# jyf588/SimGAN

Hardware: AMD Instinct MI355X
Metric: env-steps/sec of GAIL-dyn PPO update (higher is better)
Workload: dtype f32; 1 GPU; northstar: GAIL-dyn update, T=128 N=512/GPU obs=47 act=12 D-in=86 policy=mlp h64 D h100 ppo_epoch=10 num_mini_batch=1...; optimizer_steps_per_update=2720, parallelism=single GPU

## Files before the change

### simgan_amd/csrc/sg_disc_step4.hpp

```cpp
#pragma once

struct Step4Args {
    PregatherArgs next;
    double* loss_acc;
};

#define SG_STEP4_TIMEOUT_TICKS 300000000ll

__device__ __forceinline__ float sg_ld_sc1(__amdgpu_buffer_rsrc_t r, int byte_off) {
    return __uint_as_float(__builtin_amdgcn_raw_buffer_load_b32(r, byte_off, 0, 16 ));
}

__device__ __forceinline__ bool sg_step4_wait(const unsigned* flags, int lo, int hi, unsigned want, int lane) {
    const long long deadline = wall_clock64() + SG_STEP4_TIMEOUT_TICKS;
    for (int it = 0;; ++it) {
        bool ok = true;
        for (int j = lo + lane; j < hi; j += 64) ok = ok & (__hip_atomic_load(flags + j * SG_STEP4_FLAG_STRIDE, __ATOMIC_RELAXED, __HIP_MEMORY_SCOPE_AGENT) == want);
        if (__all(ok)) return true;
        if ((it & 31) == 31 && wall_clock64() > deadline) return false;
        __builtin_amdgcn_s_sleep(1);
    }
}

template <int KF, int KH>
__global__ __launch_bounds__(512) void k_disc_step4(float* c_params, float* c_m, float* c_v, float* c_wT, float* c_ops,
                                                   SgOptState* c_st, int c_pack ,
                                                   int c_B, Step4Args a) {
    constexpr int Fp = 16 * KF, Hp = 16 * KH, ldF = Fp + 4, ldH = Hp + 4;
    constexpr int NWC = KF > KH ? KF : KH;
    constexpr int W_LDS = 8 * 256, C_LDS = SG_CHAIN4_LDS_FLOATS(KF, KH);
    __shared__ __attribute__((aligned(16))) float sm[(C_LDS > W_LDS ? C_LDS : W_LDS) + 4];
    const int c_G = c_pack & 1023, c_k1 = (int)((unsigned)c_pack >> 14);
    const int tid = threadIdx.x, wave = tid >> 6, lane = tid & 63;
    const int Kt = 64 * c_G, n_chain = 12 * c_G, w_base = (n_chain + 7) & ~7;
    unsigned* flags = reinterpret_cast<unsigned*>(c_st) + SG_STEP4_FLAG_WORD0;
    float* c_part = c_ops + (size_t)(2 - ((c_k1 - 1) & 1)) * ((size_t)Kt * (3 * Hp + ldF + Fp));

    if ((int)blockIdx.x < n_chain) {
        if (wave >= NWC) return;
        int t0 = 0;
        if (tid == 0) t0 = c_st->t0;
        Chain4Args ca{c_params, c_wT, c_ops, c_part, c_B, c_G, 1.0f / (float)c_B, 10.0f};
        sg_chain4_body<KF, KH, true>(ca, sm);
        asm volatile("s_waitcnt vmcnt(0)" ::: "memory");
        __syncthreads();
        if (tid == 0) __hip_atomic_store(flags + blockIdx.x * SG_STEP4_FLAG_STRIDE, (unsigned)(t0 + c_k1), __ATOMIC_RELAXED, __HIP_MEMORY_SCOPE_AGENT);
        return;
    }
    const int wb = (int)blockIdx.x - w_base;
    constexpr int th = KH, tf = KF, T2 = th * th, ntv = 8 * (th + tf), NV = (3 * Hp + 4 + 63) / 64;
    static_assert((8 - th) * (th + tf) > NV, "k_disc_step4: a spare slot must exist for the Adam-scalar lane");
    if (wb < 0) return;
    if (wb >= ntv) {
        if (a.next.ops) sg_disc_pregather(a.next, wb - ntv);
        return;
    }
    SgDiscDesc d;
    d.F = 0; d.Hd = 0; d.Hp = Hp; d.Fp = Fp; d.ldF = ldF; d.ldH = ldH;
    d.w1 = 0; d.b1 = Hp * ldF; d.w2 = d.b1 + Hp; d.b2 = d.w2 + Hp * ldH; d.w3 = d.b2 + Hp; d.b3 = d.w3 + Hp; d.total = d.b3 + 16;
    float (*red)[256] = reinterpret_cast<float (*)[256]>(sm);
    int* sh_ok = reinterpret_cast<int*>(sm + W_LDS);
    unsigned* err = reinterpret_cast<unsigned*>(c_st) + SG_STEP4_ERR_WORD;
    const int xcd = wb & 7, slot = wb >> 3;
    const int li = lane & 15, lq = lane >> 4;
    constexpr int nw = 8;
    if (xcd < th) {
        const int b = slot < th ? xcd * th + slot : T2 + xcd * tf + (slot - th);
        const bool w2 = b < T2;
        const int t = w2 ? b : b - T2;
        const int tm = w2 ? t / th : t / tf, tn = w2 ? t % th : t % tf;
        const int ldp = w2 ? ldH : ldF;
        const int idx = (w2 ? d.w2 : d.w1) + (tm * 16 + ((tid & 255) >> 4)) * ldp + tn * 16 + (tid & 15);
        float p0 = 0.f, m0 = 0.f, v0 = 0.f;
        float4 sc = float4{0.f, 0.f, 1.f, 1.f};
        int t0 = 0;
        if (tid < 256) {
            p0 = c_params[idx]; m0 = c_m[idx]; v0 = c_v[idx];
            sc = *reinterpret_cast<const float4*>(c_st->step_size2);
        }
        if (tid < 256 || wave == 7) t0 = c_st->t0;
        const SgStacks stk = sg_disc_stacks(c_ops, Kt, Hp, Fp, ldF);
        const float* L = (w2 ? stk.L2 : stk.L1) + (size_t)tm * Kt * 16;
        const float* Rr = (w2 ? stk.R2 : stk.R1t) + (size_t)tn * Kt * 16;
        const int n_chunks = Kt >> 4;
        const __amdgpu_buffer_rsrc_t rL = __builtin_amdgcn_make_buffer_rsrc(const_cast<float*>(L), 0, Kt * 64, 0x00020000);
        const __amdgpu_buffer_rsrc_t rR = __builtin_amdgcn_make_buffer_rsrc(const_cast<float*>(Rr), 0, Kt * 64, 0x00020000);
        int img0 = 0, img1 = 0;
        sg_disc_img_pos(d, w2, tm * 16 + ((tid & 255) >> 4), tn * 16 + (tid & 15), img0, img1);
        if (tid == 0) *sh_ok = 1;
        __syncthreads();
        const unsigned want = (unsigned)(t0 + c_k1);
        if (wave == 7 && (__hip_atomic_load(err, __ATOMIC_RELAXED, __HIP_MEMORY_SCOPE_AGENT) != 0 || !sg_step4_wait(flags, 4 * c_G, n_chain, want, lane)) && lane == 0) *sh_ok = 0;
        __syncthreads();
        if (!*sh_ok) { if (tid == 0) { atomicOr(err, 1u); a.loss_acc[0] = __builtin_nanf(""); } return; }
        f32x4 acc = f32x4{0.f, 0.f, 0.f, 0.f}, alt = acc;
        const int half_chunks = n_chunks >> 1;
        auto contract = [&](int c_lo, int c_hi, auto&& between) {
            bool first = true;
            for (int c0 = c_lo + wave; c0 < c_hi || first; c0 += 2 * nw) {
                float x[2][4], y[2][4];
#pragma unroll
                for (int cc = 0; cc < 2; ++cc)
#pragma unroll
                    for (int s = 0; s < 4; ++s) {
                        const int c = c0 + cc * nw;
                        const int r = c < c_hi ? 16 * c + 4 * s + lq : Kt;
                        x[cc][s] = sg_ld_sc1(rL, (r * 16 + li) * 4);
                        y[cc][s] = sg_ld_sc1(rR, (r * 16 + li) * 4);
                    }
                if (first) { between(); first = false; }
#pragma unroll
                for (int cc = 0; cc < 2; ++cc)
#pragma unroll
                    for (int s = 0; s < 4; ++s) {
                        if (s & 1) alt = sg_mfma(x[cc][s], y[cc][s], alt);
                        else acc = sg_mfma(x[cc][s], y[cc][s], acc);
                    }
            }
        };
        contract(0, half_chunks, [&]() {
            if (wave == 7 && !sg_step4_wait(flags, 0, 4 * c_G, want, lane) && lane == 0) *sh_ok = 0;
        });
        __syncthreads();
        if (!*sh_ok) { if (tid == 0) { atomicOr(err, 1u); a.loss_acc[0] = __builtin_nanf(""); } return; }
        contract(half_chunks, n_chunks, []() {});
        acc += alt;
#pragma unroll
        for (int r = 0; r < 4; ++r) red[wave][(4 * lq + r) * 16 + li] = acc[r];
        __syncthreads();
        if (tid < 256) {
            float g = 0.f;
            {
                float r8[8];
#pragma unroll
                for (int w = 0; w < 8; ++w) r8[w] = red[w][tid];
#pragma unroll
                for (int w = 0; w < 8; ++w) g += r8[w];
            }
            const bool odd = (t0 + c_k1) & 1;
            const float step_size = odd ? sc.y : sc.x, bc2_sqrt = odd ? sc.w : sc.z;
            m0 = m0 + (g - m0) * (float)(1.0 - 0.9);
            v0 = v0 * (float)0.999 + (float)(1.0 - 0.999) * g * g;
            const float denom = sqrtf(v0) / bc2_sqrt + SG_DISC_ADAM_EPS;
            p0 = p0 - step_size * (m0 / denom);
            __builtin_amdgcn_sched_barrier(0);
            __builtin_nontemporal_store(p0, c_params + idx);
            __builtin_nontemporal_store(m0, c_m + idx);
            __builtin_nontemporal_store(v0, c_v + idx);
            __builtin_nontemporal_store(p0, c_wT + img0);
            __builtin_nontemporal_store(p0, c_wT + img1);
        }
        return;
    }
    const int vid = (xcd - th) * (th + tf) + slot;
    if (vid > NV) return;
    if (vid == NV) {
        if (tid == 0) sg_opt_prepare(c_st, c_st->t0 + c_k1 + 1);
        return;
    }
    {
        const int nparts = n_chain, stride = 4 * Hp, NE = 3 * Hp + 4;
        const int i = 64 * vid + lane;
        const float4 sc = *reinterpret_cast<const float4*>(c_st->step_size2);
        const int t0 = c_st->t0;
        const bool odd = (t0 + c_k1) & 1;
        const float step_size = odd ? sc.y : sc.x, bc2_sqrt = odd ? sc.w : sc.z;
        const bool is_param = wave == 0 && i < 3 * Hp + 1;
        const int pidx = i < Hp ? d.b1 + i : i < 2 * Hp ? d.b2 + (i - Hp) : i < 3 * Hp ? d.w3 + (i - 2 * Hp) : d.b3;
        float pv = 0.f, pm = 0.f, pvv = 0.f;
        if (is_param) { pv = c_params[pidx]; pm = c_m[pidx]; pvv = c_v[pidx]; }
        const __amdgpu_buffer_rsrc_t rP = __builtin_amdgcn_make_buffer_rsrc(c_part, 0, nparts * stride * 4, 0x00020000);
        if (tid == 0) *sh_ok = 1;
        __syncthreads();
        if (wave == 7 && (__hip_atomic_load(err, __ATOMIC_RELAXED, __HIP_MEMORY_SCOPE_AGENT) != 0 || !sg_step4_wait(flags, 0, n_chain, (unsigned)(t0 + c_k1), lane)) && lane == 0) *sh_ok = 0;
        __syncthreads();
        if (!*sh_ok) { if (tid == 0) { atomicOr(err, 1u); a.loss_acc[0] = __builtin_nanf(""); } return; }
        float g = 0.f;
        if (i < NE) {
            for (int s0 = wave; s0 < nparts; s0 += 16 * nw) {
                float tt[16];
#pragma unroll
                for (int u = 0; u < 16; ++u) {
                    const int sidx = s0 + u * nw;
                    tt[u] = sidx < nparts ? sg_ld_sc1(rP, (sidx * stride + i) * 4) : 0.f;
                }
#pragma unroll
                for (int u = 0; u < 16; ++u) g += tt[u];
            }
        }
        red[wave][lane] = g;
        __syncthreads();
        if (wave == 0 && i < NE) {
            g = 0.f;
            {
                float r8[8];
#pragma unroll
                for (int w = 0; w < 8; ++w) r8[w] = red[w][lane];
#pragma unroll
                for (int w = 0; w < 8; ++w) g += r8[w];
            }
            if (i < 3 * Hp + 1) {
                pm = pm + (g - pm) * (float)(1.0 - 0.9);
                pvv = pvv * (float)0.999 + (float)(1.0 - 0.999) * g * g;
                const float denom = sqrtf(pvv) / bc2_sqrt + SG_DISC_ADAM_EPS;
                c_params[pidx] = pv - step_size * (pm / denom);
                c_m[pidx] = pm;
                c_v[pidx] = pvv;
            }
            const int l0 = (3 * Hp) & 63;
            const float el_s = __shfl(g, l0 + 1), pl_s = __shfl(g, l0 + 2), gp_s = __shfl(g, l0 + 3);
            if (i == 3 * Hp) {
                const float inv_B = 1.0f / (float)c_B;
                const float el = el_s * inv_B, pl = pl_s * inv_B, gp = 10.0f * (gp_s * inv_B);
                a.loss_acc[0] += (double)(el + pl + gp);
                a.loss_acc[1] += (double)el;
                a.loss_acc[2] += (double)pl;
            }
        }
    }
}
```

Measured before the change: 2.489 million env-steps/s.

## Split flag polling across two waves and prefetch contraction batches before waits

Wave 6 now polls the second flag group (after a short delay, using pipelined sc1 global loads) while wave 7 polls the first, and the two report through workgroup-scope LDS words instead of block-wide __syncthreads. Other waves spin on those words, issue their first operand loads as soon as the first group is ready, and then load the second batch, so global latency overlaps the cross-block wait. The second half's chunk assignment is rotated per wave. This adds inline-asm polling, spin loops on LDS words and more register pressure from the held prefetch buffers.

```diff
diff --git a/simgan_amd/csrc/sg_disc_step4.hpp b/simgan_amd/csrc/sg_disc_step4.hpp
--- a/simgan_amd/csrc/sg_disc_step4.hpp
+++ b/simgan_amd/csrc/sg_disc_step4.hpp
@@ -20,6 +20,40 @@
         if ((it & 31) == 31 && wall_clock64() > deadline) return false;
         __builtin_amdgcn_s_sleep(1);
     }
+}
+
+#define SG_STEP4_POLLS 1
+#define SG_STEP4_POLL_START_TICKS 340
+struct SgStep4Polls { unsigned r[SG_STEP4_POLLS] = {}; };
+__device__ __forceinline__ unsigned sg_step4_poll(const unsigned* p) {
+    unsigned r;
+    asm volatile("global_load_dword %0, %1, off sc1" : "=v"(r) : "v"(p) : "memory");
+    return r;
+}
+__device__ __forceinline__ bool sg_step4_wait_piped(SgStep4Polls& pp, const unsigned* flags, int n, unsigned want, int lane, const int* quit) {
+    constexpr int K = SG_STEP4_POLLS;
+    static_assert(K >= 1 && K <= 3, "SG_STEP4_POLLS: 1, 2 or 3");
+    const unsigned* p = flags + (lane < n ? lane : n - 1) * SG_STEP4_FLAG_STRIDE;
+    const long long deadline = wall_clock64() + SG_STEP4_TIMEOUT_TICKS;
+#pragma unroll
+    for (int i = 0; i < K; ++i) {
+        pp.r[i] = sg_step4_poll(p);
+        if (i + 1 < K) __builtin_amdgcn_s_sleep(28 / K);
+    }
+    for (int it = 0;; ++it) {
+#pragma unroll
+        for (int i = 0; i < K; ++i) {
+            asm volatile("s_waitcnt vmcnt(%1)" : "+v"(pp.r[i]) : "n"(K - 1) : "memory");
+            if (__all(pp.r[i] == want)) return true;
+            __builtin_amdgcn_s_sleep(1);
+            pp.r[i] = sg_step4_poll(p);
+        }
+        if ((it & 31) == 31 && (wall_clock64() > deadline || __hip_atomic_load(quit, __ATOMIC_RELAXED, __HIP_MEMORY_SCOPE_WORKGROUP) == 2)) return false;
+    }
+}
+__device__ __forceinline__ void sg_step4_polls_retire(SgStep4Polls& pp) {
+#pragma unroll
+    for (int i = 0; i < SG_STEP4_POLLS; ++i) asm volatile("" : "+v"(pp.r[i]) : : "memory");
 }
 
 template <int KF, int KH>
@@ -78,7 +112,7 @@
             p0 = c_params[idx]; m0 = c_m[idx]; v0 = c_v[idx];
             sc = *reinterpret_cast<const float4*>(c_st->step_size2);
         }
-        if (tid < 256 || wave == 7) t0 = c_st->t0;
+        if (tid < 256 || wave >= 6) t0 = c_st->t0;
         const SgStacks stk = sg_disc_stacks(c_ops, Kt, Hp, Fp, ldF);
         const float* L = (w2 ? stk.L2 : stk.L1) + (size_t)tm * Kt * 16;
         const float* Rr = (w2 ? stk.R2 : stk.R1t) + (size_t)tn * Kt * 16;
@@ -87,46 +121,92 @@
         const __amdgpu_buffer_rsrc_t rR = __builtin_amdgcn_make_buffer_rsrc(const_cast<float*>(Rr), 0, Kt * 64, 0x00020000);
         int img0 = 0, img1 = 0;
         sg_disc_img_pos(d, w2, tm * 16 + ((tid & 255) >> 4), tn * 16 + (tid & 15), img0, img1);
-        if (tid == 0) *sh_ok = 1;
+        const int half_chunks = n_chunks >> 1;
+        auto batch_offs = [&](int c0, int c_hi, int (&o)[2][4]) {
+#pragma unroll
+            for (int cc = 0; cc < 2; ++cc)
+#pragma unroll
+                for (int s = 0; s < 4; ++s) {
+                    const int c = c0 + cc * nw;
+                    const int r = c < c_hi ? 16 * c + 4 * s + lq : Kt;
+                    o[cc][s] = (r * 16 + li) * 4;
+                }
+        };
+        const int mix0 = half_chunks + ((wave - half_chunks) & (nw - 1));
+        int oa[2][4], ob[2][4];
+        batch_offs(wave, half_chunks, oa);
+        batch_offs(mix0, n_chunks, ob);
+#pragma unroll
+        for (int cc = 0; cc < 2; ++cc)
+#pragma unroll
+            for (int s = 0; s < 4; ++s) asm volatile("" : "+v"(oa[cc][s]), "+v"(ob[cc][s]));
+        int* sh_bce = sh_ok + 1;
+        int* sh_mix = sh_ok + 2;
+        if (tid == 0) { *sh_bce = 0; *sh_mix = 0; }
+        const long long poll_from = wall_clock64() + SG_STEP4_POLL_START_TICKS;
         __syncthreads();
         const unsigned want = (unsigned)(t0 + c_k1);
-        if (wave == 7 && (__hip_atomic_load(err, __ATOMIC_RELAXED, __HIP_MEMORY_SCOPE_AGENT) != 0 || !sg_step4_wait(flags, 4 * c_G, n_chain, want, lane)) && lane == 0) *sh_ok = 0;
-        __syncthreads();
-        if (!*sh_ok) { if (tid == 0) { atomicOr(err, 1u); a.loss_acc[0] = __builtin_nanf(""); } return; }
+        auto word_set = [&](int* w, bool up) {
+            if (lane == 0) __hip_atomic_store(w, up ? 1 : 2, __ATOMIC_RELAXED, __HIP_MEMORY_SCOPE_WORKGROUP);
+        };
+        auto word_up = [&](int* w) -> bool {
+            int s;
+            while ((s = __hip_atomic_load(w, __ATOMIC_RELAXED, __HIP_MEMORY_SCOPE_WORKGROUP)) == 0) __builtin_amdgcn_s_sleep(1);
+            asm volatile("" ::: "memory");
+            return s == 1;
+        };
+        SgStep4Polls pp;
+        if (wave == 7) {
+            word_set(sh_bce, __hip_atomic_load(err, __ATOMIC_RELAXED, __HIP_MEMORY_SCOPE_AGENT) == 0 && sg_step4_wait(flags, 4 * c_G, n_chain, want, lane));
+        } else if (wave == 6) {
+            bool up = __hip_atomic_load(err, __ATOMIC_RELAXED, __HIP_MEMORY_SCOPE_AGENT) == 0;
+            if (up) {
+                while (wall_clock64() < poll_from) __builtin_amdgcn_s_sleep(2);
+                up = 4 * c_G <= 64 ? sg_step4_wait_piped(pp, flags, 4 * c_G, want, lane, sh_bce) : sg_step4_wait(flags, 0, 4 * c_G, want, lane);
+            }
+            word_set(sh_mix, up);
+        }
         f32x4 acc = f32x4{0.f, 0.f, 0.f, 0.f}, alt = acc;
-        const int half_chunks = n_chunks >> 1;
-        auto contract = [&](int c_lo, int c_hi, auto&& between) {
-            bool first = true;
-            for (int c0 = c_lo + wave; c0 < c_hi || first; c0 += 2 * nw) {
-                float x[2][4], y[2][4];
-#pragma unroll
-                for (int cc = 0; cc < 2; ++cc)
-#pragma unroll
-                    for (int s = 0; s < 4; ++s) {
-                        const int c = c0 + cc * nw;
-                        const int r = c < c_hi ? 16 * c + 4 * s + lq : Kt;
-                        x[cc][s] = sg_ld_sc1(rL, (r * 16 + li) * 4);
-                        y[cc][s] = sg_ld_sc1(rR, (r * 16 + li) * 4);
-                    }
-                if (first) { between(); first = false; }
-#pragma unroll
-                for (int cc = 0; cc < 2; ++cc)
-#pragma unroll
-                    for (int s = 0; s < 4; ++s) {
-                        if (s & 1) alt = sg_mfma(x[cc][s], y[cc][s], alt);
-                        else acc = sg_mfma(x[cc][s], y[cc][s], acc);
-                    }
-            }
-        };
-        contract(0, half_chunks, [&]() {
-            if (wave == 7 && !sg_step4_wait(flags, 0, 4 * c_G, want, lane) && lane == 0) *sh_ok = 0;
-        });
-        __syncthreads();
-        if (!*sh_ok) { if (tid == 0) { atomicOr(err, 1u); a.loss_acc[0] = __builtin_nanf(""); } return; }
-        contract(half_chunks, n_chunks, []() {});
+        auto load_offs = [&](const int (&o)[2][4], float (&x)[2][4], float (&y)[2][4]) {
+#pragma unroll
+            for (int cc = 0; cc < 2; ++cc)
+#pragma unroll
+                for (int s = 0; s < 4; ++s) {
+                    x[cc][s] = sg_ld_sc1(rL, o[cc][s]);
+                    y[cc][s] = sg_ld_sc1(rR, o[cc][s]);
+                }
+        };
+        auto load_batch = [&](int c0, int c_hi, float (&x)[2][4], float (&y)[2][4]) {
+            int o[2][4];
+            batch_offs(c0, c_hi, o);
+            load_offs(o, x, y);
+        };
+        auto mma_batch = [&](const float (&x)[2][4], const float (&y)[2][4]) {
+#pragma unroll
+            for (int cc = 0; cc < 2; ++cc)
+#pragma unroll
+                for (int s = 0; s < 4; ++s) {
+                    if (s & 1) alt = sg_mfma(x[cc][s], y[cc][s], alt);
+                    else acc = sg_mfma(x[cc][s], y[cc][s], acc);
+                }
+        };
+        float xa[2][4], ya[2][4], xb[2][4], yb[2][4];
+        bool up = word_up(sh_bce);
+        if (up) {
+            load_offs(oa, xa, ya);
+            up = word_up(sh_mix);
+        }
+        if (!up) { if (tid == 0) { atomicOr(err, 1u); a.loss_acc[0] = __builtin_nanf(""); } return; }
+        load_offs(ob, xb, yb);
+        __builtin_amdgcn_sched_barrier(0);
+        mma_batch(xa, ya);
+        for (int c0 = wave + 2 * nw; c0 < half_chunks; c0 += 2 * nw) { load_batch(c0, half_chunks, xa, ya); mma_batch(xa, ya); }
+        mma_batch(xb, yb);
+        for (int c0 = mix0 + 2 * nw; c0 < n_chunks; c0 += 2 * nw) { load_batch(c0, n_chunks, xb, yb); mma_batch(xb, yb); }
         acc += alt;
 #pragma unroll
         for (int r = 0; r < 4; ++r) red[wave][(4 * lq + r) * 16 + li] = acc[r];
+        sg_step4_polls_retire(pp);
         __syncthreads();
         if (tid < 256) {
             float g = 0.f;
```

After: 2.554 million env-steps/s (median of 6 runs). 1.03x the previous value.
